# pgriewank/SAMSIM

Hardware: NVIDIA B200
Metric: column-timesteps/sec (FP64, 100 layers) (higher is better)
Workload: dtype f64

## Files before the change

samsim_b200/csrc/physics.cuh:

```cuda
#pragma once

#include <stdint.h>

#include "detmath.h"
#include "params.cuh"

namespace samsim {

struct DevCfg {
  int testcase;
  int Nlayer, N_top, N_middle, N_bottom;
  int atmoflux_flag, grav_flag, prescribe_flag, grav_heat_flag, flush_heat_flag, turb_flag, salt_flag,
      boundflux_flag, flush_flag, flood_flag, bottom_flag, precip_flag, harmonic_flag, tank_flag, albedo_flag,
      lab_snow_flag, freeboard_snow_flag, snow_flush_flag, snow_precip_flag;
  int i_time_out;
  int n_bgc;
  double dt, thick_0, thick_min, time_out;
  double alpha_flux_instable, alpha_flux_stable, m_total;
  double max_flux_plate, k_snow_flush, k_styropor;
  double c2, c3, c4, d2, d3x2, d4x3;
  int two_pass;
  int pf;
};

#ifdef SAMSIM_HOST_BUILD
static const DevCfg* samsim_host_cfg = nullptr;
#define CFG (*samsim::samsim_host_cfg)
#else
__constant__ DevCfg samsim_dev_cfg;
#define CFG samsim::samsim_dev_cfg
#endif

enum {
  SC_T_BOTTOM = 0, SC_T_TOP, SC_S_BU_BOTTOM, SC_T2M, SC_FL_Q_BOTTOM,
  SC_PSI_S_SNOW, SC_PSI_L_SNOW, SC_PSI_G_SNOW, SC_PHI_S, SC_S_ABS_SNOW, SC_H_ABS_SNOW, SC_M_SNOW, SC_T_SNOW,
  SC_THICK_SNOW, SC_LIQUID_PRECIP, SC_SOLID_PRECIP, SC_FL_Q_SNOW,
  SC_ENERGY_STORED, SC_TOTAL_RESIST, SC_FRESHWATER, SC_THICKNESS, SC_BULK_SALIN,
  SC_ALBEDO, SC_FL_SW, SC_FL_LW, SC_FL_REST,
  SC_GRAV_DRAIN, SC_GRAV_SALT, SC_GRAV_TEMP,
  SC_MELT_THICK, SC_MELT_THICK_SNOW, SC_MELT_THICK_SNOW_OLD,
  SC_MTO1, SC_MTO2, SC_MTO3,
  SC_FREEBOARD, SC_T_FREEZE, SC_MELT_ERR, SC_S_TOTAL,
  SC_TTOP_WARM, SC_TTOP_COLD, SC_OFLUX_AMP,
  SC_BGC_BOTTOM1, SC_BGC_BOTTOM2, SC_BGC_TOTAL1, SC_BGC_TOTAL2,
  SC_COUNT
};
enum {
  AR_M = 0, AR_S_ABS, AR_H_ABS, AR_THICK, AR_T, AR_PHI, AR_S_BU, AR_PSI_S, AR_PSI_L, AR_PSI_G, AR_RAY, AR_PERM,
  AR_FLUSH_V, AR_FLUSH_H, AR_FL_Q,
  AR_STATE_COUNT,
  AR_S_BR = AR_STATE_COUNT, AR_V_EX, AR_FL_M, AR_W0, AR_W1, AR_W2, AR_W3,
  AR_CORE_COUNT,
  AR_BGC1 = AR_CORE_COUNT, AR_BGC2, AR_FB_D, AR_FB_U, AR_FB_A, AR_FB_O,
  AR_COUNT
};
enum { IN_N_ACTIVE = 0, IN_STATUS, IN_STYROPOR, IN_EVENTS0, IN_EVENTS1, IN_COUNT };

enum {
  EV_FLOOD = 0, EV_FLOOD_NEG_FREE, EV_FLOOD_SIMPLE, EV_FLUSH3, EV_FLUSH4, EV_FLUSH_INLINE, EV_STYROPOR, EV_SNOW_THERMO,
  EV_SNOW_THERMO_MELTWATER, EV_SNOW_WET, EV_SNOW_MERGE, EV_SNOW_COMPACTION, EV_SNOW_COUPLING_ITER,
  EV_SNOW_COUPLING_WARM1, EV_SNOW_COUPLING_WARM2, EV_SNOW_PRECIP, EV_SNOW_PRECIP_0, EV_MELT_SNOW_ALL, EV_MELT_SNOW_PART,
  EV_BOTTOM_MELT, EV_BOTTOM_MELT_SIMPLE_A, EV_BOTTOM_MELT_SIMPLE_B, EV_BOTTOM_GROWTH_SIMPLE, EV_BOTTOM_GROWTH,
  EV_TOP_GROW_A, EV_TOP_GROW_B, EV_TOP_GROW_C, EV_TOP_MELT_A, EV_TOP_MELT_B, EV_TOP_MELT_C, EV_GRAV_DRAINED,
  EV_SALT_CLAMP,
  EV_GAS_REFILL, EV_GETT_TFR_FALLBACK, EV_GETT_SALTFREE, EV_GETT_LIQUID, EV_HEAT_MELT, EV_HEAT_THIN_SNOW,
  EV_MELT_THICK_GAS, EV_SNOW_MELTWATER_TO_ICE, EV_PRESCRIBE, EV_GRAV_DRAIN_SIMPLE, EV_NOTZFLUX, EV_FLUSH3_CLAMP,
  EV_SCRUB, EV_MELT_THICK, EV_TURB, EV_TANK, EV_TWO_PASS_STEP,
  EV_COUNT
};

struct Lay {
  double* p;
  unsigned ls;
  __device__ __forceinline__ double& operator[](int k) const {
#if !defined(SAMSIM_HOST_BUILD) && defined(__CUDA_ARCH__)
    __builtin_assume(__isGlobal(p));
#endif
    return p[(unsigned)k * ls];
  }
  __device__ __forceinline__ void prefetch(int k) const {
#ifndef SAMSIM_HOST_BUILD
    asm volatile("prefetch.global.L1 [%0];" ::"l"(p + (unsigned)k * ls));
#else
    (void)k;
#endif
  }
};
#ifndef SAMSIM_LOOP
#define SAMSIM_LOOP _Pragma("unroll 1")
#endif
#ifndef SAMSIM_PF
#define SAMSIM_PF (CFG.pf)
#endif

#define SAMSIM_TILE 32
struct View {
  double* base;
  unsigned ls;
  __device__ __forceinline__ Lay A(int id) const { return Lay{base + id * SAMSIM_TILE, ls}; }
  __device__ __forceinline__ Lay m() const { return A(AR_M); }
  __device__ __forceinline__ Lay S_abs() const { return A(AR_S_ABS); }
  __device__ __forceinline__ Lay H_abs() const { return A(AR_H_ABS); }
  __device__ __forceinline__ Lay thick() const { return A(AR_THICK); }
  __device__ __forceinline__ Lay T() const { return A(AR_T); }
  __device__ __forceinline__ Lay phi() const { return A(AR_PHI); }
  __device__ __forceinline__ Lay S_bu() const { return A(AR_S_BU); }
  __device__ __forceinline__ Lay psi_s() const { return A(AR_PSI_S); }
  __device__ __forceinline__ Lay psi_l() const { return A(AR_PSI_L); }
  __device__ __forceinline__ Lay psi_g() const { return A(AR_PSI_G); }
  __device__ __forceinline__ Lay ray() const { return A(AR_RAY); }
  __device__ __forceinline__ Lay perm() const { return A(AR_PERM); }
  __device__ __forceinline__ Lay flush_v() const { return A(AR_FLUSH_V); }
  __device__ __forceinline__ Lay flush_h() const { return A(AR_FLUSH_H); }
  __device__ __forceinline__ Lay fl_Q() const { return A(AR_FL_Q); }
  __device__ __forceinline__ Lay S_br() const { return A(AR_S_BR); }
  __device__ __forceinline__ Lay V_ex() const { return A(AR_V_EX); }
  __device__ __forceinline__ Lay fl_m() const { return A(AR_FL_M); }
  __device__ __forceinline__ Lay w0() const { return A(AR_W0); }
  __device__ __forceinline__ Lay w1() const { return A(AR_W1); }
  __device__ __forceinline__ Lay w2() const { return A(AR_W2); }
  __device__ __forceinline__ Lay w3() const { return A(AR_W3); }
  __device__ __forceinline__ Lay bgc(int q) const { return A(AR_BGC1 + q); }
};
struct Col : View {
  double fb_x;
  int N_active, status, styropor_flag;
  unsigned ev0, ev1;
  bool thermo_valid;
  bool want_state;
  struct FbMemo {
    bool tot_valid;  double t1, A, G;
    bool suf_valid;  int ks; double As, Gs;
    bool res_valid;  double m1, th1, msnow, result;
    int k_last;
  } fb;
  double min_psi_s, min_S_abs_2;
  struct Pre {
    bool valid;
    double mn2, sq2, st2;
    double bottom_h, S_br_Na, perm_Na;
    double A2;
  } pre;
  double sc[SC_COUNT];
  double time;
  long long i;
  int n_time_out, time_counter;
  double fsw0, fsw1, flw0, flw1;
  double ftime0, ftime1;
// ... 549 lines not shown
    m1 = m1 + m_snow;
    thick1 = thick1 + thick_snow;
    H_abs_snow = 0.0; m_snow = 0.0; thick_snow = 0.0;
    psi_g_snow = 0.0; psi_s_snow = 0.0; psi_l_snow = 0.0;
  }
  if (psi_g_snow < 0.0) c.status = 9876;
}

__device__ __forceinline__ void snow_block(Col& c) {
  const View v = c;
  if (SCV(c, SC_THICK_SNOW) > 0.0) {
    double m1 = v.m()[1], th1 = v.thick()[1], H1 = v.H_abs()[1];
    if (CFG.snow_flush_flag == 0) {
      double dummy = 0.0;
      snow_thermo(c, false, m1, th1, H1, dummy);
      SCV(c, SC_MELT_THICK_SNOW) = 0.0;
    } else if (CFG.snow_flush_flag == 1) {
      SCV(c, SC_MELT_THICK_SNOW) = 0.0;
      snow_thermo(c, true, m1, th1, H1, SCV(c, SC_MELT_THICK_SNOW));
    }
    v.m()[1] = m1; v.thick()[1] = th1; v.H_abs()[1] = H1;
  } else {
    SCV(c, SC_THICK_SNOW) = 0.0; SCV(c, SC_M_SNOW) = 0.0; SCV(c, SC_PSI_S_SNOW) = 0.0; SCV(c, SC_PSI_L_SNOW) = 0.0;
    SCV(c, SC_PSI_G_SNOW) = 0.0; SCV(c, SC_H_ABS_SNOW) = 0.0; SCV(c, SC_S_ABS_SNOW) = 0.0;
    SCV(c, SC_MELT_THICK_SNOW) = 0.0;
  }
}

__device__ __forceinline__ double fl_Q_0_snow_thin(double m_snow, double thick_snow, double T_snow, double ps,
                                                   double pl, double pg, double thick, double T_bound) {
  double ks = k_snow_of(m_snow, thick_snow);
  double k = ps * k_s + pl * k_l + pg * 0.0;
  k = thick_snow / (thick_snow + thick) * ks + thick / (thick_snow + thick) * k;
  double R = (thick_snow + thick) / (2.0 * k);
  return (T_snow - T_bound) / R;
}
__device__ __forceinline__ double fl_Q_snow_ice(double m_snow, double thick_snow, double T_snow, double ps2,
                                                double pl2, double th2, double T2) {
  double ks = k_snow_of(m_snow, thick_snow);
  double k2 = ps2 * k_s + pl2 * k_l;
  double R = thick_snow / (2.0 * ks) + th2 / (2.0 * k2);
  return (T2 - T_snow) / R;
}
__device__ __forceinline__ double fl_Q_0_snow(double m_snow, double thick_snow, double T_snow, double T_bound) {
  double k = k_snow_of(m_snow, thick_snow);
  double R = thick_snow / (2.0 * k);
  return (T_snow - T_bound) / R;
}


#ifndef SAMSIM_GB
#define SAMSIM_GB 8
#endif
__device__ __noinline__ void grav_drain(Col& c, bool exact_all) {
  const View v = c;
  const int Na = c.N_active, N = CFG.Nlayer;
  const double dt = CFG.dt;
  Lay q = v.w1(), smin = v.w2(), fl_m = v.fl_m();
  double heat_loss = 0.0;

  SAMSIM_LOOP
  for (int k = Na; k <= N - 1; k++) v.ray()[k] = 0.0;
  const double bottom_h = v.thick()[Na] * v.psi_s()[Na] / psi_s_min;
  const double S_br_Na = v.S_br()[Na];
  double perm_Na = 0.0;
  int kmin_cand = 0, ncand = 0;
  {
    double mn = 0.0, sq = 0.0, st = 0.0, st_below = 0.0, qb_est = 0.0;
    SAMSIM_LOOP
    for (int k = Na; k >= 1; k--) {
      if (k - SAMSIM_PF >= 1) { v.psi_l().prefetch(k - SAMSIM_PF); v.thick().prefetch(k - SAMSIM_PF); v.S_br().prefetch(k - SAMSIM_PF); }
      const double pk = 1e-17 * det_pow(1000.0 * fabs(v.psi_l()[k]), 3.10);
      if (k == Na) { perm_Na = pk; qb_est = bottom_h / pk; continue; }
      const double thk = v.thick()[k];
      const double qk = thk / pk;
      q[k] = qk;
      mn = (k == Na - 1) ? pk : f_min(mn, pk);
      if (exact_all) {
        smin[k] = mn;
      } else {
        st_below = st;
        sq = sq + qk;
        st = st + thk;
        double est;
        if (CFG.harmonic_flag == 1) {
          est = grav * rho_l * bbeta * (v.S_br()[k] - S_br_Na) * (st_below + bottom_h) * f_min(mn, perm_Na);
          smin[k] = mn;
        } else {
          const double hp = (mn < 1e-14) ? 0.0 : (st + bottom_h) / (sq + qb_est);
          est = grav * rho_l * bbeta * (v.S_br()[k] - S_br_Na) * (st_below + bottom_h) * hp;
        }
        est = est / (kappa_l * mu);
        const double rest = (CFG.harmonic_flag == 2 && mn < 1e-14) ? 0.0 : f_max(est, 0.0);
        v.ray()[k] = rest;
        if (rest > ray_crit * (1.0 - 1e-10)) { kmin_cand = k; ncand++; }
      }
    }
  }
  const double qb = bottom_h / perm_Na;

  const bool blocked = exact_all || ncand >= 3;
  const int kstop = exact_all ? 1 : kmin_cand;
  int kexact_from = exact_all ? 1 : Na;
  double carry_t = 0.0;
  for (int k0 = ((Na - 2) / SAMSIM_GB) * SAMSIM_GB + 1; blocked && k0 >= 1 && k0 + SAMSIM_GB - 1 >= kstop && Na >= 2; k0 -= SAMSIM_GB) {
    kexact_from = k0;
    double aq[SAMSIM_GB], at[SAMSIM_GB];
#pragma unroll
    for (int j = 0; j < SAMSIM_GB; j++) { aq[j] = 0.0; at[j] = 0.0; }
    SAMSIM_LOOP
    for (int d = 0; d < SAMSIM_GB; d++) {
      const int kk = k0 + d;
      if (kk <= Na - 1) {
        const double qv = q[kk], tv = v.thick()[kk];
#pragma unroll
        for (int j = 0; j < SAMSIM_GB; j++) {
          const double nq = aq[j] + qv, nt = at[j] + tv;
          aq[j] = (j <= d) ? nq : aq[j];
          at[j] = (j <= d) ? nt : at[j];
        }
      }
    }
    SAMSIM_LOOP
    for (int kk = k0 + SAMSIM_GB; kk <= Na - 1; kk++) {
      if (kk + 8 <= Na - 1) { q.prefetch(kk + 8); v.thick().prefetch(kk + 8); }
      const double qv = q[kk], tv = v.thick()[kk];
#pragma unroll
      for (int j = 0; j < SAMSIM_GB; j++) { aq[j] = aq[j] + qv; at[j] = at[j] + tv; }
    }
    const double carry_next = at[0];
    double below = carry_t;
    SAMSIM_LOOP
    for (int j = SAMSIM_GB - 1; j >= 0; j--) {
      const int k = k0 + j;
      const double aqj = aq[SAMSIM_GB - 1], atj = at[SAMSIM_GB - 1];
#pragma unroll
      for (int i = SAMSIM_GB - 1; i >= 1; i--) { aq[i] = aq[i - 1]; at[i] = at[i - 1]; }
      if (k <= Na - 1) {
        const double height = below + bottom_h;
        const double d_S_br = v.S_br()[k] - S_br_Na;
        double r;
        if (CFG.harmonic_flag == 1) {
          r = grav * rho_l * bbeta * d_S_br * height * f_min(smin[k], perm_Na);
        } else {
          const bool zero = exact_all ? (smin[k] < 1e-14) : (v.ray()[k] == 0.0);
          double hp;
          if (zero) {
            hp = 0.0;
          } else {
            hp = aqj + qb;
            hp = (atj + bottom_h) / hp;
          }
          r = grav * rho_l * bbeta * d_S_br * height * hp;
        }
        r = r / (kappa_l * mu);
        v.ray()[k] = f_max(r, 0.0);
      }
      below = atj;
    }
    carry_t = carry_next;
  }

  double sum_before = 0.0, sum_after = 0.0;
  double min_S = 1e300;
  int kfirst = 0;

  double run = 0.0;
  double sbk = v.S_br()[1];
  SAMSIM_LOOP
  for (int k = 1; k <= Na - 1; k++) {
    if (k + SAMSIM_PF <= Na) {
      v.ray().prefetch(k + SAMSIM_PF); v.S_abs().prefetch(k + SAMSIM_PF); v.S_br().prefetch(k + SAMSIM_PF);
    }
    double rk = v.ray()[k];
    const double Sk = v.S_abs()[k];
    const double sbk1 = v.S_br()[k + 1];
    if (k < kexact_from && rk > ray_crit * (1.0 - 1e-10)) {
      double hq = 0.0, ht = 0.0, hb = 0.0;
      SAMSIM_LOOP
      for (int kk = k; kk <= Na - 1; kk++) {
        const double tv = v.thick()[kk];
        hq = hq + q[kk];
        ht = ht + tv;
        if (kk > k) hb = hb + tv;
      }
      const double height = hb + bottom_h;
      const double d_S_br = sbk - S_br_Na;
      double r;
      if (CFG.harmonic_flag == 1) {
        r = grav * rho_l * bbeta * d_S_br * height * f_min(smin[k], perm_Na);
      } else {
        double hp = hq + qb;
        hp = (ht + bottom_h) / hp;
        r = grav * rho_l * bbeta * d_S_br * height * hp;
      }
      r = r / (kappa_l * mu);
      rk = f_max(r, 0.0);
      v.ray()[k] = rk;
    }
    double up = run;
    double S_after = Sk;
    double fl_down_k = 0.0;
    sum_before = sum_before + Sk;
    if (rk > ray_crit && v.psi_s()[k] > 0.001 && Sk / v.m()[k] > 0.1 && sbk > sbk1) {
      if (kfirst == 0) { kfirst = k; fl_m[k] = 0.0; EVT(c, EV_GRAV_DRAINED); }
      const double plk = v.psi_l()[k], thk = v.thick()[k], Tk = v.T()[k];
      double flux = x_grav * (rk - ray_crit) * dt * thk;
      flux = f_min(flux, plk * rho_l * thk);
      fl_down_k = flux;
      double Snew = Sk - flux * sbk;
      v.S_abs()[k] = Snew;
      S_after = Snew;
      if (Snew < 0.0) { c.status = 21234; return; }
      SCV(c, SC_GRAV_TEMP) = SCV(c, SC_GRAV_TEMP) + flux * Tk;
      v.H_abs()[k] = v.H_abs()[k] - flux * c_l * Tk;
      heat_loss = heat_loss + flux * c_l * Tk;
      run = run + flux;
      up = f_min(run, plk * rho_l * thk);
    }
    if (CFG.n_bgc) {
      const double cellNa = (k == Na - 1) ? v.A(AR_FB_D)[k] : v.A(AR_FB_A)[k];
      v.A(AR_FB_O)[k] = cellNa + fl_down_k;
      v.A(AR_FB_U)[k] = v.A(AR_FB_U)[k] + up;
    }
    if (kfirst) fl_m[k + 1] = up;
    else min_S = f_min(min_S, Sk);
    sum_after = sum_after + S_after;
    sbk = sbk1;
  }
  if (kfirst) fl_m[Na + 1] = run;
  if (CFG.n_bgc) v.A(AR_FB_U)[Na] = v.A(AR_FB_U)[Na] + run;
  const double fl_up_Na = run;
  {
    const double S_Na = v.S_abs()[Na];
    sum_before = sum_before + S_Na;
    sum_after = sum_after + S_Na;
  }
  SCV(c, SC_GRAV_SALT) = SCV(c, SC_GRAV_SALT) + sum_before;
  SCV(c, SC_GRAV_SALT) = SCV(c, SC_GRAV_SALT) - sum_after;

  if (kfirst) mass_transfer(c, fl_m, v.S_bu(), kfirst);

  SCV(c, SC_GRAV_DRAIN) = SCV(c, SC_GRAV_DRAIN) + run;
  if (CFG.grav_heat_flag == 2) v.H_abs()[Na] = v.H_abs()[Na] + heat_loss - fl_up_Na * c_l * SCV(c, SC_T_BOTTOM);
  double mn = min_S;
  if (kfirst) for (int k = kfirst; k <= Na; k++) mn = f_min(mn, v.S_abs()[k]);
  else mn = f_min(mn, v.S_abs()[Na]);
  if (f_min(mn, 0.0) < 0.0) c.status = 1337;
}

__device__ __noinline__ void grav_drain_simple(Col& c) {
  const View v = c;
  const int Na = c.N_active, N = CFG.Nlayer;
  Lay perm = v.w0(), hperm = v.w2();
  SAMSIM_LOOP
  for (int k = 1; k <= N - 1; k++) v.ray()[k] = 0.0;
  SAMSIM_LOOP
  for (int k = 1; k <= Na; k++) perm[k] = 1e-17 * det_pow(1000.0 * fabs(v.psi_l()[k]), 3.10);
  const double bottom_h = v.thick()[Na] * v.psi_s()[Na] / psi_s_min;
  if (CFG.harmonic_flag == 2) {
    SAMSIM_LOOP
    for (int k = 1; k <= Na - 1; k++) {
      double mn = perm[k];
      SAMSIM_LOOP
      for (int kk = k; kk <= Na - 1; kk++) mn = f_min(mn, perm[kk]);
      if (mn < 1e-14) {
        hperm[k] = 0.0;
      } else {
        double h = 0.0;
        SAMSIM_LOOP
        for (int kk = k; kk <= Na - 1; kk++) h = h + v.thick()[kk] / perm[kk];
        h = h + bottom_h / perm[Na];
        hperm[k] = (sum_fwd(v.thick(), k, Na - 1) + bottom_h) / h;
      }
    }
  }
  const double S_br_Na = v.S_br()[Na];
  SAMSIM_LOOP
  for (int k = 1; k <= Na - 1; k++) {
// ... 809 lines not shown
```

samsim_b200/csrc/samsim_b200.cu:

```cuda
#include <cuda_runtime.h>
#include <math.h>
#include <stdint.h>
#include <stdio.h>
#include <string.h>

#include <string>
#include <vector>

#include <cub/device/device_radix_sort.cuh>

#include "../../include/samsim_b200.h"
#include "step.cuh"

using namespace samsim;

static_assert((int)SAMSIM_SC_COUNT == (int)SC_COUNT, "scalar ids out of sync with include/samsim_b200.h");
static_assert((int)SAMSIM_ARR_COUNT == (int)AR_STATE_COUNT + 2 && (int)SAMSIM_ARR_BGC_ABS1 == (int)AR_STATE_COUNT,
              "array ids out of sync with include/samsim_b200.h");
static_assert((int)SAMSIM_INT_COUNT == (int)IN_COUNT, "int ids out of sync with include/samsim_b200.h");
static_assert((int)SAMSIM_EV_COUNT == (int)EV_COUNT && (int)SAMSIM_EV_TWO_PASS_STEP == (int)EV_TWO_PASS_STEP && (int)SAMSIM_EV_GAS_REFILL == 32,
              "event ids out of sync with include/samsim_b200.h");
static_assert((int)SAMSIM_SNAPSC_COUNT == 20 && (int)SAMSIM_SNAPARR_COUNT == 14, "snapshot layout");

#ifndef SAMSIM_BLOCK
// ... 34 lines not shown
  asm volatile("cp.async.ca.shared.global [%0], [%1], 8;\n" ::"r"(s), "l"(gmem_src));
}

template <bool TWO_PASS>
__global__ void __launch_bounds__(SAMSIM_BLOCK, SAMSIM_MINBLOCKS) samsim_step_kernel(const __grid_constant__ KParams p) {
  __shared__ double s_win[SAMSIM_MAXSITE * 4 * SAMSIM_MAXWIN];
  if (p.series != nullptr) {
    const int n = p.nsite * 4 * p.win_len;
    for (int e = threadIdx.x; e < n; e += blockDim.x) {
      const int sk = e / p.win_len, r = e - sk * p.win_len;
      cp_async8(&s_win[e], p.series + (size_t)sk * p.nrec + (p.win_first - 1 + r));
    }
    asm volatile("cp.async.commit_group;\n" ::);
    asm volatile("cp.async.wait_group 0;\n" ::);
  }
  __syncthreads();

  const long long col_raw = (long long)blockIdx.x * blockDim.x + threadIdx.x;
  const bool padding = (col_raw >= p.ncol);
  const long long col = padding ? (p.ncol - 1) : col_raw;
  const size_t ls = (size_t)p.ncol_pad;

  Col c;
  c.ls = (unsigned)(p.n_arr * SAMSIM_TILE);
  c.base = p.arr + (size_t)(col / SAMSIM_TILE) * p.LS * c.ls + (size_t)(col % SAMSIM_TILE);
  for (int q = 0; q < SC_COUNT; q++) c.sc[q] = p.sc[(size_t)q * ls + col];
  c.N_active = p.in[(size_t)IN_N_ACTIVE * ls + col];
  c.status = padding ? -1 : p.in[(size_t)IN_STATUS * ls + col];
  c.styropor_flag = p.in[(size_t)IN_STYROPOR * ls + col];
  c.ev0 = (unsigned)p.in[(size_t)IN_EVENTS0 * ls + col];
  c.ev1 = (unsigned)p.in[(size_t)IN_EVENTS1 * ls + col];
  c.time = p.time; c.i = p.i; c.n_time_out = p.n_time_out; c.time_counter = p.time_counter;
  c.fsw0 = c.fsw1 = c.flw0 = c.flw1 = c.ftime0 = c.ftime1 = 0.0;
  c.thermo_valid = false;
  c.pre.valid = false;
  c.want_state = false;
  c.fb.tot_valid = c.fb.suf_valid = c.fb.res_valid = false; c.fb.k_last = 0; c.fb.ks = 0;
  c.min_psi_s = 0.0; c.min_S_abs_2 = 0.0;
  c.fb_x = 0.0;

  Forcing f;
  f.win = s_win; f.win_len = p.win_len; f.win_first = p.win_first;
  f.site = p.site_of_col ? p.site_of_col[col] : 0;
  for (int k = 0; k < 4; k++) {
    f.scale[k] = p.fscale ? p.fscale[(size_t)k * ls + col] : 1.0;
    f.offset[k] = p.foffset ? p.foffset[(size_t)k * ls + col] : 0.0;
  }
  f.lab = p.lab; f.lab_nrec = p.lab_nrec;
  f.lab_set = p.set_of_col ? p.set_of_col[col] : 0;

  SnapOut snap;
  snap.scalars = p.snap_sc; snap.arrays = p.snap_arr; snap.ncol_pad = ls; snap.col = (int)col;

  for (int s = 0; s < p.nsteps; s++) column_step<TWO_PASS>(c, f, s == p.nsteps - 1, snap);

  if (p.divergence) {
    const unsigned full = 0xffffffffu;
    const bool live = !padding && c.status == 0;
    const int na = live ? c.N_active : 0;
    const int mx = __reduce_max_sync(full, na);
    const int idle = __reduce_add_sync(full, live ? (mx - na) : 0);
    const int nlive = __popc(__ballot_sync(full, live));
    const double ts = c.sc[SC_THICK_SNOW];
    const int cls = !live ? -1 : (((ts <= 0.0) ? 0 : (ts < CFG.thick_min / 100.0) ? 1 : (ts < CFG.thick_min) ? 2 : 3) |
                                  ((c.sc[SC_MELT_THICK] > 0.0) ? 4 : 0));
    const int cls0 = __shfl_sync(full, cls, __ffs(__ballot_sync(full, live)) - 1);
    const unsigned differ = __ballot_sync(full, live && cls != cls0);
    if ((threadIdx.x & 31) == 0 && nlive > 0) {
      atomicAdd(&p.divergence[0], (unsigned long long)idle);
      atomicAdd(&p.divergence[1], (unsigned long long)mx * (unsigned long long)nlive);
      atomicAdd(&p.divergence[2], (unsigned long long)(differ != 0u));
      atomicAdd(&p.divergence[3], 1ull);
    }
  }

  if (padding) return;
  for (int q = 0; q < SC_COUNT; q++) p.sc[(size_t)q * ls + col] = c.sc[q];
  p.in[(size_t)IN_N_ACTIVE * ls + col] = c.N_active;
  p.in[(size_t)IN_STATUS * ls + col] = c.status;
  p.in[(size_t)IN_STYROPOR * ls + col] = c.styropor_flag;
  p.in[(size_t)IN_EVENTS0 * ls + col] = (int)c.ev0;
  p.in[(size_t)IN_EVENTS1 * ls + col] = (int)c.ev1;
}

__device__ __forceinline__ long long slot_of(const int* map, long long col) { return map ? (long long)map[col] : col; }

__host__ __device__ __forceinline__ size_t state_index(long long s, int k, int a, int LS, int n_arr) {
  return ((((size_t)(s / SAMSIM_TILE)) * LS + k) * n_arr + a) * SAMSIM_TILE + (size_t)(s % SAMSIM_TILE);
}

__global__ void samsim_broadcast_kernel(double* arr, double* sc, int* in, long long ncol_pad, int LS, int src, int col0,
                                        int n, const int* map, int n_arr) {
  const long long t = (long long)blockIdx.x * blockDim.x + threadIdx.x;
  if (t >= n) return;
  const long long col = slot_of(map, col0 + t);
  src = (int)slot_of(map, src);
  if (col == src) return;
  const size_t ls = (size_t)ncol_pad;
  for (int k = 0; k < LS; k++)
    for (int a = 0; a < n_arr; a++) arr[state_index(col, k, a, LS, n_arr)] = arr[state_index(src, k, a, LS, n_arr)];
  for (int q = 0; q < SC_COUNT; q++) sc[(size_t)q * ls + col] = sc[(size_t)q * ls + src];
  for (int q = 0; q < IN_COUNT; q++) in[(size_t)q * ls + col] = in[(size_t)q * ls + src];
}

__global__ void samsim_gather_kernel(const double* src, double* dst, long long ncol_pad, int LS, int count, int ext,
                                     int col0, int n, int k0, const int* map) {
  const long long t = (long long)blockIdx.x * blockDim.x + threadIdx.x;
// ... 1064 lines not shown
  int rc = kat_common(device);
  if (rc) return rc;
  if (n < 1 || !a || !out) return fail(SAMSIM_ERR_ARG, "kat_scalar: bad argument");
  if ((rc = kat_upload_cfg(device, salt_flag))) return rc;
  double* d = nullptr;
  const size_t nb = (size_t)n * sizeof(double);
  CU(cudaMalloc(&d, 3 * nb));
  CU(cudaMemcpy(d, a, nb, cudaMemcpyHostToDevice));
  if (b) CU(cudaMemcpy(d + n, b, nb, cudaMemcpyHostToDevice));
  else CU(cudaMemset(d + n, 0, nb));
  samsim_kat_scalar_kernel<<<(n + 127) / 128, 128>>>(fn, salt_flag, n, d, d + n, d + 2 * (size_t)n);
  CU(cudaGetLastError());
  CU(cudaMemcpy(out, d + 2 * (size_t)n, nb, cudaMemcpyDeviceToHost));
  cudaFree(d);
  return 0;
}

int samsim_b200_fp64_peak(int32_t device, double seconds, double* tflops) {
  int rc = kat_common(device);
  if (rc) return rc;
  if (!tflops) return fail(SAMSIM_ERR_ARG, "fp64_peak: bad argument");
  cudaDeviceProp prop;
  CU(cudaGetDeviceProperties(&prop, device));
  const int blocks = prop.multiProcessorCount * 8, threads = 256;
  double* d = nullptr;
  CU(cudaMalloc(&d, (size_t)blocks * threads * sizeof(double)));
  cudaEvent_t e0, e1;
  cudaEventCreate(&e0);
  cudaEventCreate(&e1);
  int iters = 2000;
  double best = 0.0, elapsed_total = 0.0;
  samsim_fp64_peak_kernel<<<blocks, threads>>>(d, 100, 1.0);
  CU(cudaDeviceSynchronize());
  while (elapsed_total < seconds * 1000.0) {
    cudaEventRecord(e0);
    samsim_fp64_peak_kernel<<<blocks, threads>>>(d, iters, 1.0);
    cudaEventRecord(e1);
    CU(cudaEventSynchronize(e1));
    float ms = 0.f;
    cudaEventElapsedTime(&ms, e0, e1);
    elapsed_total += ms;
    const double flop = 2.0 * 64.0 * (double)iters * blocks * threads;
    const double tf = flop / (ms * 1e-3) / 1e12;
    if (tf > best) best = tf;
    if (ms < 50.f) iters *= 2;
  }
  cudaEventDestroy(e0);
  cudaEventDestroy(e1);
  cudaFree(d);
  *tflops = best;
  return 0;
}

}
```

samsim_b200/csrc/step.cuh:

```cuda
#pragma once

#include "physics.cuh"

namespace samsim {

struct Forcing {
  const double* win;
  int win_len;
  int win_first;
  int site;
  double scale[4], offset[4];
  const double* lab;
  long long lab_nrec;
  int lab_set;
};

__device__ __forceinline__ double forcing_rec(const Forcing& f, int kind, int rec ) {
  const double base = f.win[(f.site * 4 + kind) * f.win_len + (rec - f.win_first)];
  return base * f.scale[kind] + f.offset[kind];
}
__device__ __forceinline__ double time_input(int k) { return ((double)(float)k - 1.0) * 3600.0 * 3.0; }
__device__ __forceinline__ double lab_rec(const Forcing& f, int kind, long long rec ) {
  return f.lab[((long long)(f.lab_set * 4 + kind)) * f.lab_nrec + (rec - 1)];
}
// ... 201 lines not shown
      }
      double fq_kp1;
      double hr_n = 0.0, T_n = 0.0;
      if (k < Na) {
        const double ps_n = v.psi_s()[k + 1], pl_n = v.psi_l()[k + 1], th_n = v.thick()[k + 1];
        T_n = v.T()[k + 1];
        hr_n = th_n / (2.0 * (ps_n * k_s + pl_n * k_l + 0.0 * 0.0));
        const double R = hr_k + hr_n;
        fq_kp1 = (T_n - T_k) / R;
        if (c.want_state) v.fl_Q()[k + 1] = fq_kp1;
      } else {
        fq_kp1 = fl_q_bottom;
      }
      double H = v.H_abs()[k];
      temp1 = temp1 + H;
      H = H + (fq_kp1 - fq_k) * dt;
      H = H + rad;
      v.H_abs()[k] = H;
      temp2 = temp2 + H;
      fq_k = fq_kp1;
      hr_k = hr_n; T_k = T_n;
    }
    temp1 = temp1 + SCV(c, SC_H_ABS_SNOW);
    SAMSIM_LOOP
    for (int k = 1; k <= Na; k++) temp1 = temp1 + rad;
  }

  bool layer1_changed = false;
  if (thick_snow >= thick_min / 100.0 && thick_snow < thick_min) {
    EVT(c, EV_HEAT_THIN_SNOW);
    SCV(c, SC_H_ABS_SNOW) = SCV(c, SC_H_ABS_SNOW) - fl_q_snow * dt;
    double H1 = v.H_abs()[1], phi1 = v.phi()[1];
    snow_coupling(c, H1, phi1, T1, v.m()[1], v.S_bu()[1]);
    v.H_abs()[1] = H1; v.phi()[1] = phi1; v.T()[1] = T1;
    layer1_changed = true;
    temp1 = temp1 + fl_q_bottom * dt - fl_q_snow * dt;
  } else if (thick_snow >= thick_min) {
    SCV(c, SC_H_ABS_SNOW) = SCV(c, SC_H_ABS_SNOW) + (flQ1 - fl_q_snow) * dt;
    temp1 = temp1 + fl_q_bottom * dt - fl_q_snow * dt;
  } else {
    temp1 = temp1 + fl_q_bottom * dt - flQ1 * dt;
  }
  if (layer1_changed) temp2 = sum_fwd(v.H_abs(), 1, Na);
  temp2 = temp2 + SCV(c, SC_H_ABS_SNOW);
  if (fabs((temp1 - temp2) / dt) > 0.00001) c.status = 431;
}

#ifndef SAMSIM_SYNC
#define SAMSIM_SYNC 1
#endif
#ifndef SAMSIM_ALWAYS_STORE_S_BU
#define SAMSIM_ALWAYS_STORE_S_BU false
#endif
#if SAMSIM_SYNC
#define SAMSIM_PHASE_SYNC() __syncthreads()
#else
#define SAMSIM_PHASE_SYNC() ((void)0)
#endif
#if SAMSIM_SYNC >= 2
#error "SAMSIM_SYNC=2 (a barrier per layer of the Newton sweeps) was removed: it measured slower and its fused / unfused \
choice per thread made the barrier divergent (ADVICE round 1)"
#endif

struct SnapOut {
  double* scalars;
  double* arrays;
  size_t ncol_pad;
  int col;
};

__device__ __noinline__ void write_snapshot(const Col& c, const SnapOut& s) {
  const View v = c;
  if (s.scalars) {
    const int ids[19] = {SC_FREEBOARD, SC_THICK_SNOW, SC_T_SNOW, SC_PSI_L_SNOW, SC_PSI_S_SNOW, SC_ENERGY_STORED,
                         SC_FRESHWATER, SC_TOTAL_RESIST, SC_THICKNESS, SC_BULK_SALIN, SC_GRAV_DRAIN, SC_GRAV_SALT,
                         SC_GRAV_TEMP, SC_T2M, SC_T_TOP, SC_MTO1, SC_MTO2, SC_MTO3, -1};
    SAMSIM_LOOP
    for (int q = 0; q < 18; q++) s.scalars[(size_t)q * s.ncol_pad + s.col] = c.sc[ids[q]];
    s.scalars[(size_t)18 * s.ncol_pad + s.col] = c.time;
    s.scalars[(size_t)19 * s.ncol_pad + s.col] = (double)c.N_active;
  }
  if (s.arrays) {
    const int N = CFG.Nlayer;
    const size_t LS = (size_t)(N + 2);
    const int src[10] = {AR_T, AR_PSI_S, AR_THICK, AR_S_BU, AR_RAY, AR_PSI_L, AR_PERM, AR_FLUSH_V, AR_FLUSH_H, AR_PSI_G};
    SAMSIM_LOOP
    for (int a = 0; a < 10; a++) {
      double* dst = s.arrays + ((size_t)a * LS) * s.ncol_pad + s.col;
      const Lay from = v.A(src[a]);
      const int n = (a == 4) ? N - 1 : N;
      SAMSIM_LOOP
      for (int k = 1; k <= n; k++) dst[(size_t)k * s.ncol_pad] = from[k];
    }
    for (int q = 0; q < CFG.n_bgc; q++) {
      double* bu = s.arrays + ((size_t)(10 + 2 * q) * LS) * s.ncol_pad + s.col;
      double* br = s.arrays + ((size_t)(11 + 2 * q) * LS) * s.ncol_pad + s.col;
      const Lay x = v.bgc(q);
      const double bottom = c.sc[SC_BGC_BOTTOM1 + q];
      SAMSIM_LOOP
      for (int k = 1; k <= N; k++) {
        double vbu = bottom, vbr = bottom;
        if (k <= c.N_active) {
          const double mk = v.m()[k];
          if (mk != 0.0) {
            vbu = x[k] / mk;
            const double pl = v.psi_l()[k], th = v.thick()[k];
            vbr = (pl != 0.0 && th != 0.0) ? x[k] / pl / th / rho_l : 0.0;
          } else {
            vbu = 0.0; vbr = 0.0;
          }
        }
        bu[(size_t)k * s.ncol_pad] = vbu;
        br[(size_t)k * s.ncol_pad] = vbr;
      }
    }
  }
}

__device__ __noinline__ void fused_thermo_expulsion(Col& c) {
  const View v = c;
  const int Na = c.N_active;
  const bool transfer = (c.i != 1);
  {
    const double m1 = v.m()[1];
    const double sbu1 = v.S_abs()[1] / m1, H = v.H_abs()[1] / m1;
    double phi1 = v.phi()[1], T1;
    const double T_test = (Na >= 2) ? v.T()[2] : SCV(c, SC_T_BOTTOM);
    getT(H, sbu1, T_test, T1, phi1, c.status, c.ev1);
    v.T()[1] = T1; v.phi()[1] = phi1;
  }
  double T_km1 = 0.0, sbr_km1 = 0.0, Sabs_km1 = 0.0, f0 = 0.0;
  double fbA = 0.0, fbG = 0.0, fbAs = 0.0, fbGs = 0.0;
  const int ks = (c.fb.k_last >= 1 && c.fb.k_last < Na) ? c.fb.k_last : 0;
  double min_ps = 1e300;
  SAMSIM_LOOP
  for (int k = 1; k <= Na; k++) {
    if (k + SAMSIM_PF <= Na) {
      v.T().prefetch(k + SAMSIM_PF); v.phi().prefetch(k + SAMSIM_PF);
      v.m().prefetch(k + SAMSIM_PF); v.thick().prefetch(k + SAMSIM_PF); v.S_abs().prefetch(k + SAMSIM_PF);
      v.H_abs().prefetch(k + SAMSIM_PF);
    }
    const double thk = v.thick()[k], m_k = v.m()[k], T_k = v.T()[k];
    double S = v.S_abs()[k];
    const double sbr_k = S_br_of(T_k, S / m_k);
    v.S_br()[k] = sbr_k;
    double ps, pl, pg, vex;
    expulsion(v.phi()[k], thk, m_k, ps, pl, pg, vex);
    double f1;
    if (k == 1) {
      f1 = -vex * rho_l;
    } else if (pg < SAMSIM_F32(0.001)) {
      f1 = -vex * rho_l + f0;
    } else {
      f1 = -f_max((vex - pg * thk) * rho_l, 0.0);
      pg = f_max((pg * thk - vex) / thk, 0.0);
    }
    v.psi_s()[k] = ps; v.psi_l()[k] = pl; v.psi_g()[k] = pg;
    fbA = fbA + ps * thk;
    fbG = fbG + pg * thk;
    if (ks && k > ks) { fbAs = fbAs + ps * thk; fbGs = fbGs + pg * thk; }
    min_ps = f_min(min_ps, ps);
    const double m_new = m_k + f1 - f0;
    v.m()[k] = m_new;
    if (transfer) {
      double H = v.H_abs()[k];
      if (f1 < 0.) {
        H = H + f1 * T_k * c_l;
        S = S + f_max(f1 * sbr_k, -S);
      }
      if (f0 < 0) {
        H = H - f0 * T_km1 * c_l;
        S = S - f_max(f0 * sbr_km1, -Sabs_km1);
      }
      v.H_abs()[k] = H;
      v.S_abs()[k] = S;
    }
    v.S_bu()[k] = S / m_new;
    if (CFG.n_bgc) {
      v.A(AR_FB_D)[k] = transfer ? -f1 : 0.0;
      v.A(AR_FB_U)[k] = 0.0; v.A(AR_FB_A)[k] = 0.0; v.A(AR_FB_O)[k] = 0.0;
    }
    T_km1 = T_k; sbr_km1 = sbr_k; Sabs_km1 = S;
    f0 = f1;
  }
  c.fb.tot_valid = true; c.fb.t1 = v.thick()[1]; c.fb.A = fbA; c.fb.G = fbG;
  c.fb.suf_valid = (ks != 0); c.fb.ks = ks; c.fb.As = fbAs; c.fb.Gs = fbGs;
  c.fb.res_valid = false;
  c.min_psi_s = min_ps;
}

__device__ __forceinline__ void testcase_hooks(Col& c, const Forcing& f) {
  const View v = c;
  const double dt = CFG.dt;
  const int N = CFG.Nlayer;
  if (CFG.testcase == 1) {
    const double j = rint(c.time / 43200.0);
    if (j >= 1.0 && j <= 20.0 && fabs(c.time - 12.0 * j * 3600.0) < SAMSIM_F32(0.01))
      SCV(c, SC_T_TOP) = (((int)j) & 1) ? SCV(c, SC_TTOP_COLD) : SCV(c, SC_TTOP_WARM);
  } else if (CFG.testcase >= 101 && CFG.testcase <= 105) {
    const long long idx = (long long)floor(1 + c.time / dt);
    const double Sb = v.S_bu()[c.N_active + 1];
    SCV(c, SC_T2M) = lab_rec(f, 0, idx);
    SCV(c, SC_SOLID_PRECIP) = lab_rec(f, 1, idx);
    SCV(c, SC_FL_Q_BOTTOM) = lab_rec(f, 2, idx);
    SCV(c, SC_T_BOTTOM) = -SAMSIM_F32(0.0575) * Sb + SAMSIM_F32(1.710523e-3) * det_pow(Sb, 3.0 / 2.0) -
                          SAMSIM_F32(2.154996e-4) * P2(Sb) - SAMSIM_F32(7.53e-4) * sum_fwd(v.thick(), 1, c.N_active - 1);
    c.styropor_flag = (int)lab_rec(f, 3, idx);
  } else if (CFG.testcase == 4 || CFG.testcase == 7) {
    const double amp = SCV(c, SC_OFLUX_AMP);
    SCV(c, SC_FL_Q_BOTTOM) = -amp * det_sin(c.time * (2.0 * pi_sp) / (86400.0 * 365.0)) + amp;
  } else if (CFG.testcase == 2) {
    if (c.time > 86400.0 * 25.0) SCV(c, SC_T2M) = 15.0;
    else if (c.time > 86400.0 * 15.0) SCV(c, SC_T2M) = 1.0;
  } else if (CFG.testcase == 9) {
    if (c.time < (19.75 * 3600.0)) SCV(c, SC_T2M) = 0.0;
    else if (c.time < (86400.0 * 3.0 + 2.25 * 3600.0)) SCV(c, SC_T2M) = -15.0;
    else SCV(c, SC_T2M) = 1.0;
  } else if (CFG.testcase == 34) {
    if (c.time < 2.0 * 3600.0) SCV(c, SC_T2M) = 0.0;
    else if (c.time < (86400.0 * 5.0)) SCV(c, SC_T2M) = -15.0;
    else if (c.time < (86400.0 * 7.0)) SCV(c, SC_T2M) = -5.0;
    else SCV(c, SC_T2M) = 1.0;
  } else if (CFG.testcase == 99) {
    if (c.time < 86400.0 * 3.0) {
      SCV(c, SC_T2M) = -40.0;
    } else {
      SCV(c, SC_T2M) = (c.time > 86400.0 * 5.0) ? 5.0 : -5.0;
      SCV(c, SC_THICK_SNOW) = 0.2;
      SCV(c, SC_T_SNOW) = -5.0;
      SCV(c, SC_M_SNOW) = 30.0;
// ... 405 lines not shown
        double fq_jp1, hr_n = 0.0, T_n = 0.0;
        if (j < Na) {
          const double ps_n = v.psi_s()[j + 1], pl_n = v.psi_l()[j + 1], th_n = v.thick()[j + 1];
          T_n = v.T()[j + 1];
          hr_n = th_n / (2.0 * (ps_n * k_s + pl_n * k_l + 0.0 * 0.0));
          fq_jp1 = (T_n - T_j) / (hr_j + hr_n);
        } else {
          fq_jp1 = fl_q_bottom;
        }
        double Hh = v.H_abs()[j];
        temp1 = temp1 + Hh;
        Hh = Hh + (fq_jp1 - fq_km1) * dt;
        Hh = Hh + rad;
        v.H_abs()[j] = Hh;
        temp2 = temp2 + Hh;
        fq_km1 = fq_jp1; hr_j = hr_n; T_j = T_n;
      }
    }
  }

  c.fb.tot_valid = true; c.fb.t1 = v.thick()[1]; c.fb.A = fbA; c.fb.G = fbG;
  c.fb.suf_valid = (ks != 0); c.fb.ks = ks; c.fb.As = fbAs; c.fb.Gs = fbGs;
  c.fb.res_valid = false;
  c.min_psi_s = neg_ps ? -1.0 : 1.0;

  if (!merge_heat) {
    if (c.status == 0) heat_fluxes(c);
    return;
  }
  v.fl_Q()[1] = flQ1;
  v.fl_Q()[Na + 1] = fl_q_bottom;
  temp1 = temp1 + SCV(c, SC_H_ABS_SNOW);
  SAMSIM_LOOP
  for (int kk = 1; kk <= Na; kk++) temp1 = temp1 + rad;
  if (SCV(c, SC_THICK_SNOW) >= CFG.thick_min) {
    const double fl_q_snow = SCV(c, SC_FL_Q_SNOW);
    SCV(c, SC_H_ABS_SNOW) = SCV(c, SC_H_ABS_SNOW) + (flQ1 - fl_q_snow) * dt;
    temp1 = temp1 + fl_q_bottom * dt - fl_q_snow * dt;
  } else {
    temp1 = temp1 + fl_q_bottom * dt - flQ1 * dt;
  }
  temp2 = temp2 + SCV(c, SC_H_ABS_SNOW);
  if (c.status == 0 && fabs((temp1 - temp2) / dt) > 0.00001) c.status = 431;
}

template <bool TWO_PASS>
__device__ __noinline__ void column_step(Col& c, const Forcing& f, bool want_diag, const SnapOut& snap) {
  const View v = c;
  const double dt = CFG.dt;
  const int N = CFG.Nlayer;
  c.i = c.i + 1;
  c.want_state = want_diag;
  const bool output_step = (c.n_time_out == CFG.i_time_out || c.i == 1);

  if (c.status == 0) {
  if (output_step || want_diag) vital_signs(c);

  if (CFG.atmoflux_flag == 2) {
    if (c.time > time_input(c.time_counter)) c.time_counter = c.time_counter + 1;
    const int tc = c.time_counter;
    c.ftime1 = time_input(tc);
    c.fsw1 = forcing_rec(f, 0, tc);
    c.flw1 = forcing_rec(f, 1, tc);
    if (c.time == c.ftime1) {
      SCV(c, SC_T2M) = forcing_rec(f, 2, tc);
      SCV(c, SC_LIQUID_PRECIP) = forcing_rec(f, 3, tc);
      c.ftime0 = 0.0; c.fsw0 = 0.0; c.flw0 = 0.0;
    } else {
      c.ftime0 = time_input(tc - 1);
      c.fsw0 = forcing_rec(f, 0, tc - 1);
      c.flw0 = forcing_rec(f, 1, tc - 1);
      const double temp = (c.time - c.ftime0) / (c.ftime1 - c.ftime0);
      SCV(c, SC_T2M) = (1.0 - temp) * forcing_rec(f, 2, tc - 1) + temp * forcing_rec(f, 2, tc);
      SCV(c, SC_LIQUID_PRECIP) = (1.0 - temp) * forcing_rec(f, 3, tc - 1) + temp * forcing_rec(f, 3, tc);
    }
  }
  long long lab_idx = 0;
  if (CFG.boundflux_flag == 3 && CFG.lab_snow_flag == 1) {
    lab_idx = (long long)floor(1 + c.time / dt);
    SCV(c, SC_SOLID_PRECIP) = lab_rec(f, 1, lab_idx);
  }

  {
    const double lp = SCV(c, SC_LIQUID_PRECIP), sp = SCV(c, SC_SOLID_PRECIP);
    if (f_max(lp, sp) > 0.0 && (CFG.precip_flag == 1 || CFG.precip_flag == 0)) {
      const bool have_solid = (CFG.precip_flag == 0);
      if (c.N_active > 1) {
        EVT(c, EV_SNOW_PRECIP);
        snow_precip(c, dt, lp, SCV(c, SC_T2M), have_solid, sp);
      } else if (c.N_active == 1) {
        EVT(c, EV_SNOW_PRECIP_0);
        double H1 = v.H_abs()[1], S1 = v.S_abs()[1];
        snow_precip_0(H1, S1, v.m()[1], v.T()[1], dt, lp, SCV(c, SC_T2M), have_solid, sp);
        v.H_abs()[1] = H1; v.S_abs()[1] = S1;
      }
    }
  }

  snow_block(c);

  }
  SAMSIM_PHASE_SYNC();
  const bool next_step_outputs_pre = ((output_step ? 0 : c.n_time_out + 1) == CFG.i_time_out);
  const bool fast = TWO_PASS && (c.status == 0) && fast_path_ok(c, output_step, want_diag || next_step_outputs_pre);
  if (c.status == 0 && !fast) {
  if (!c.thermo_valid) backward_pass<false>(c, false, false);
  fused_thermo_expulsion(c);

  }
  SAMSIM_PHASE_SYNC();
  if (c.status == 0) {
  c.fb_x = 0.0;
  if (output_step) {
    SCV(c, SC_FREEBOARD) = (c.N_active > 1) ? freeboard_of(c) : 0.0;
    if (CFG.grav_flag == 2) {
      if (SCV(c, SC_GRAV_DRAIN) == 0.0) SCV(c, SC_GRAV_TEMP) = 0.0;
      else SCV(c, SC_GRAV_TEMP) = SCV(c, SC_GRAV_TEMP) / SCV(c, SC_GRAV_DRAIN);
      SCV(c, SC_GRAV_SALT) = SCV(c, SC_GRAV_SALT) / CFG.time_out;
      SCV(c, SC_GRAV_DRAIN) = SCV(c, SC_GRAV_DRAIN) / CFG.time_out;
    }
    write_snapshot(c, snap);
    SCV(c, SC_GRAV_DRAIN) = 0.0; SCV(c, SC_GRAV_SALT) = 0.0; SCV(c, SC_GRAV_TEMP) = 0.0;
    SCV(c, SC_MTO1) = 0.0; SCV(c, SC_MTO2) = 0.0; SCV(c, SC_MTO3) = 0.0;
    c.n_time_out = 0;
  } else {
    c.n_time_out = c.n_time_out + 1;
  }

  }
  SAMSIM_PHASE_SYNC();
  if (c.status == 0 && !fast) {
  {
    const int Na = c.N_active;
    const double pg = v.psi_g()[Na];
    if (pg > 0.0) {
      EVT(c, EV_GAS_REFILL);
      const double temp2 = pg * v.thick()[Na] * rho_l;
      c.fb.res_valid = false;
      v.m()[Na] = v.m()[Na] + temp2;
      v.S_abs()[Na] = v.S_abs()[Na] + temp2 * SCV(c, SC_S_BU_BOTTOM);
      v.H_abs()[Na] = v.H_abs()[Na] + temp2 * c_l * SCV(c, SC_T_BOTTOM);
    }
  }

  if (SCV(c, SC_M_SNOW) > 0.0 && SCV(c, SC_THICK_SNOW) < CFG.thick_min) {
    double H1 = v.H_abs()[1], phi1 = v.phi()[1], T1 = v.T()[1];
    snow_coupling(c, H1, phi1, T1, v.m()[1], v.S_bu()[1]);
    v.H_abs()[1] = H1; v.phi()[1] = phi1; v.T()[1] = T1;
    }

  if (c.N_active > 1 && CFG.flood_flag > 1) {
    SCV(c, SC_FREEBOARD) = freeboard_of(c);
    if (SCV(c, SC_FREEBOARD) < 0.0) {
      if (CFG.flood_flag == 2) { flood(c); fb_reset(c); }
      else if (CFG.flood_flag == 3 && SCV(c, SC_FREEBOARD) < neg_free) { flood_simple(c); fb_reset(c); }
    }
  }

  if (CFG.turb_flag == 2) {
    EVT(c, EV_TURB);
    const int Na = c.N_active;
    const double S = v.S_abs()[Na], mNa = v.m()[Na];
    const double turb = Turb_A * det_exp(Turb_B * (-density_of(SCV(c, SC_T_BOTTOM), SCV(c, SC_S_BU_BOTTOM)) + density_of(v.T()[Na], S / mNa))) * dt;
    v.S_abs()[Na] = S - turb * (S / mNa - SCV(c, SC_S_BU_BOTTOM));
    for (int q = 0; q < CFG.n_bgc; q++) {
      const double b = v.bgc(q)[Na];
      v.bgc(q)[Na] = b - turb * (b / mNa - SCV(c, SC_BGC_BOTTOM1 + q));
    }
  }

  }
  SAMSIM_PHASE_SYNC();
  if (TWO_PASS) {
    if (c.status == 0 && fast) {
      EVT(c, EV_TWO_PASS_STEP);
      testcase_hooks(c, f);
      forward_pass(c);
    }
  }
  if (c.status == 0 && !fast) {
  if (CFG.grav_flag == 2 && c.N_active > 1) {
    const bool next_step_outputs = (c.n_time_out == CFG.i_time_out);
    grav_drain(c, c.want_state || next_step_outputs);
  }
  else if (CFG.grav_flag == 3 && c.N_active > 1) { EVT(c, EV_GRAV_DRAIN_SIMPLE); grav_drain_simple(c); }

  if (CFG.prescribe_flag == 2) {
    EVT(c, EV_PRESCRIBE);
    const int Na = c.N_active;
    const double Sb = SCV(c, SC_S_BU_BOTTOM);
    int k = Na;
    while (k > 1 && sum_fwd(v.thick(), k, Na) < 0.15) {
      v.S_bu()[k] = Sb - sum_fwd(v.thick(), k, Na) / 0.15 * (Sb - 4.0);
      k = k - 1;
    }
    while (k > 1 && sum_fwd(v.thick(), k, Na) >= 0.15) {
      v.S_bu()[k] = 4.0 - 4.0 * (sum_fwd(v.thick(), k, Na) - 0.15) / (sum_fwd(v.thick(), 1, Na) - 0.15);
      k = k - 1;
      v.S_bu()[1] = 0.0;
    }
    v.S_bu()[Na] = Sb;
    SAMSIM_LOOP
    for (int kk = 1; kk <= N; kk++) v.S_abs()[kk] = v.S_bu()[kk] * v.m()[kk];
  }

  }
  SAMSIM_PHASE_SYNC();
  if (c.status == 0 && !fast) {
  testcase_hooks(c, f);

  if (CFG.tank_flag == 2) {
    EVT(c, EV_TANK);
    SCV(c, SC_S_BU_BOTTOM) = (SCV(c, SC_S_TOTAL) - sum_fwd(v.S_abs(), 1, c.N_active)) / (CFG.m_total - sum_fwd(v.m(), 1, c.N_active));
    if (CFG.n_bgc) {
      const double vb = (SCV(c, SC_BGC_TOTAL1) - sum_fwd(v.bgc(0), 1, c.N_active)) / (CFG.m_total - sum_fwd(v.m(), 1, c.N_active));
      for (int q = 0; q < CFG.n_bgc; q++) SCV(c, SC_BGC_BOTTOM1 + q) = vb;
    }
  }

  heat_fluxes(c);

  }
  SAMSIM_PHASE_SYNC();
  if (c.status == 0) {
  {
    const bool next_step_outputs = (c.n_time_out == CFG.i_time_out);
    const bool prepare = TWO_PASS && !(c.want_state || next_step_outputs) && c.N_active >= 3 && CFG.grav_flag == 2 &&
                         CFG.harmonic_flag == 2 && CFG.n_bgc == 0;
    backward_pass<TWO_PASS>(c, prepare, c.want_state || SAMSIM_ALWAYS_STORE_S_BU);
  }

  }
  SAMSIM_PHASE_SYNC();
  if (c.status == 0) {
  SCV(c, SC_MELT_THICK_SNOW_OLD) = SCV(c, SC_MELT_THICK_SNOW);
  snow_block(c);
// ... 130 lines not shown
```

Before: 120.5 million.

## Defer S_bu stores to grav_drain and skip undrained layers in flux loop

Outside output, prescribe and bgc steps, fused_thermo_expulsion no longer writes bulk salinity for interior layers. grav_drain writes S_bu only for layers from the first drained one downward, which cuts per-layer global stores. When there are no bgc tracers, grav_drain also runs a light loop over layers above the lowest Rayleigh candidate that only accumulates salt sums, skipping ray/S_br loads. The change also adds optional phase-cycle and host traffic-count instrumentation behind compile flags. The risk is that S_bu is left stale in undrained interior layers, which is correct only if nothing reads it before the next output step.

```diff
diff --git a/samsim_b200/csrc/physics.cuh b/samsim_b200/csrc/physics.cuh
--- a/samsim_b200/csrc/physics.cuh
+++ b/samsim_b200/csrc/physics.cuh
@@ -69,15 +69,33 @@
   EV_COUNT
 };
 
+#if defined(SAMSIM_HOST_BUILD) && defined(SAMSIM_COUNT_TRAFFIC)
+#define SAMSIM_TRAFFIC_PHASES 16
+static const double* samsim_traffic_base = nullptr;
+static int samsim_traffic_phase = 0;
+static long long samsim_traffic[SAMSIM_TRAFFIC_PHASES][AR_COUNT][2];
+inline void samsim_traffic_count(const double* e, int w);
+struct LayRef {
+  double* e;
+  operator double() const { samsim_traffic_count(e, 0); return *e; }
+  const LayRef& operator=(double x) const { samsim_traffic_count(e, 1); *e = x; return *this; }
+  const LayRef& operator=(const LayRef& o) const { return *this = (double)o; }
+};
+#endif
+
 struct Lay {
   double* p;
   unsigned ls;
+#if defined(SAMSIM_HOST_BUILD) && defined(SAMSIM_COUNT_TRAFFIC)
+  LayRef operator[](int k) const { return LayRef{p + (unsigned)k * ls}; }
+#else
   __device__ __forceinline__ double& operator[](int k) const {
 #if !defined(SAMSIM_HOST_BUILD) && defined(__CUDA_ARCH__)
     __builtin_assume(__isGlobal(p));
 #endif
     return p[(unsigned)k * ls];
   }
+#endif
   __device__ __forceinline__ void prefetch(int k) const {
 #ifndef SAMSIM_HOST_BUILD
     asm volatile("prefetch.global.L1 [%0];" ::"l"(p + (unsigned)k * ls));
@@ -94,6 +112,13 @@
 #endif
 
 #define SAMSIM_TILE 32
+#if defined(SAMSIM_HOST_BUILD) && defined(SAMSIM_COUNT_TRAFFIC)
+inline void samsim_traffic_count(const double* e, int w) {
+  const long long off = (e - samsim_traffic_base) / SAMSIM_TILE;
+  const int ph = samsim_traffic_phase < SAMSIM_TRAFFIC_PHASES ? samsim_traffic_phase : SAMSIM_TRAFFIC_PHASES - 1;
+  if (samsim_traffic_base && off >= 0) samsim_traffic[ph][off % AR_COUNT][w]++;
+}
+#endif
 struct View {
   double* base;
   unsigned ls;
@@ -749,7 +774,7 @@
 #ifndef SAMSIM_GB
 #define SAMSIM_GB 8
 #endif
-__device__ __noinline__ void grav_drain(Col& c, bool exact_all) {
+__device__ __noinline__ void grav_drain(Col& c, bool exact_all, bool store_S_bu) {
   const View v = c;
   const int Na = c.N_active, N = CFG.Nlayer;
   const double dt = CFG.dt;
@@ -797,10 +822,10 @@
   const double qb = bottom_h / perm_Na;
 
   const bool blocked = exact_all || ncand >= 3;
-  const int kstop = exact_all ? 1 : kmin_cand;
+  const int kc = exact_all ? 1 : (ncand ? kmin_cand : Na);
   int kexact_from = exact_all ? 1 : Na;
   double carry_t = 0.0;
-  for (int k0 = ((Na - 2) / SAMSIM_GB) * SAMSIM_GB + 1; blocked && k0 >= 1 && k0 + SAMSIM_GB - 1 >= kstop && Na >= 2; k0 -= SAMSIM_GB) {
+  for (int k0 = ((Na - 2) / SAMSIM_GB) * SAMSIM_GB + 1; blocked && k0 >= 1 && k0 + SAMSIM_GB - 1 >= kc && Na >= 2; k0 -= SAMSIM_GB) {
     kexact_from = k0;
     double aq[SAMSIM_GB], at[SAMSIM_GB];
 #pragma unroll
@@ -863,9 +888,20 @@
   int kfirst = 0;
 
   double run = 0.0;
-  double sbk = v.S_br()[1];
-  SAMSIM_LOOP
-  for (int k = 1; k <= Na - 1; k++) {
+  int k = 1;
+  if (CFG.n_bgc == 0) {
+    SAMSIM_LOOP
+    for (; k < kc; k++) {
+      if (k + SAMSIM_PF <= Na) v.S_abs().prefetch(k + SAMSIM_PF);
+      const double Sk = v.S_abs()[k];
+      sum_before = sum_before + Sk;
+      min_S = f_min(min_S, Sk);
+      sum_after = sum_after + Sk;
+    }
+  }
+  double sbk = v.S_br()[k];
+  SAMSIM_LOOP
+  for (; k <= Na - 1; k++) {
     if (k + SAMSIM_PF <= Na) {
       v.ray().prefetch(k + SAMSIM_PF); v.S_abs().prefetch(k + SAMSIM_PF); v.S_br().prefetch(k + SAMSIM_PF);
     }
@@ -900,7 +936,10 @@
     double fl_down_k = 0.0;
     sum_before = sum_before + Sk;
     if (rk > ray_crit && v.psi_s()[k] > 0.001 && Sk / v.m()[k] > 0.1 && sbk > sbk1) {
-      if (kfirst == 0) { kfirst = k; fl_m[k] = 0.0; EVT(c, EV_GRAV_DRAINED); }
+      if (kfirst == 0) {
+        kfirst = k; fl_m[k] = 0.0; EVT(c, EV_GRAV_DRAINED);
+        if (store_S_bu && k - 1 >= 2) v.S_bu()[k - 1] = v.S_abs()[k - 1] / v.m()[k - 1];
+      }
       const double plk = v.psi_l()[k], thk = v.thick()[k], Tk = v.T()[k];
       double flux = x_grav * (rk - ray_crit) * dt * thk;
       flux = f_min(flux, plk * rho_l * thk);
@@ -920,8 +959,12 @@
       v.A(AR_FB_O)[k] = cellNa + fl_down_k;
       v.A(AR_FB_U)[k] = v.A(AR_FB_U)[k] + up;
     }
-    if (kfirst) fl_m[k + 1] = up;
-    else min_S = f_min(min_S, Sk);
+    if (kfirst) {
+      fl_m[k + 1] = up;
+      if (store_S_bu && k >= 2) v.S_bu()[k] = Sk / v.m()[k];
+    } else {
+      min_S = f_min(min_S, Sk);
+    }
     sum_after = sum_after + S_after;
     sbk = sbk1;
   }
diff --git a/samsim_b200/csrc/samsim_b200.cu b/samsim_b200/csrc/samsim_b200.cu
--- a/samsim_b200/csrc/samsim_b200.cu
+++ b/samsim_b200/csrc/samsim_b200.cu
@@ -110,7 +110,19 @@
   SnapOut snap;
   snap.scalars = p.snap_sc; snap.arrays = p.snap_arr; snap.ncol_pad = ls; snap.col = (int)col;
 
+#if defined(SAMSIM_PHASE_CLOCK) && SAMSIM_SYNC
+  if (threadIdx.x == 0) {
+    for (int q = 0; q < SAMSIM_NPHASE; q++) samsim_pc_acc[q] = 0;
+    samsim_pc_ph = 0;
+  }
+  __syncthreads();
+  if (threadIdx.x == 0) samsim_pc_t0 = clock64();
+#endif
   for (int s = 0; s < p.nsteps; s++) column_step<TWO_PASS>(c, f, s == p.nsteps - 1, snap);
+#if defined(SAMSIM_PHASE_CLOCK) && SAMSIM_SYNC
+  if (threadIdx.x == 0)
+    for (int q = 0; q < SAMSIM_NPHASE; q++) atomicAdd(&samsim_phase_cycles[q], samsim_pc_acc[q]);
+#endif
 
   if (p.divergence) {
     const unsigned full = 0xffffffffu;
@@ -1281,4 +1293,15 @@
   return 0;
 }
 
-}
+#if defined(SAMSIM_PHASE_CLOCK) && SAMSIM_SYNC
+int samsim_b200_phase_cycles(unsigned long long* out) {
+  if (!out) return fail(SAMSIM_ERR_ARG, "phase_cycles: bad argument");
+  CU(cudaDeviceSynchronize());
+  CU(cudaMemcpyFromSymbol(out, samsim_phase_cycles, sizeof(unsigned long long) * SAMSIM_NPHASE));
+  const unsigned long long zero[SAMSIM_NPHASE] = {};
+  CU(cudaMemcpyToSymbol(samsim_phase_cycles, zero, sizeof zero));
+  return SAMSIM_NPHASE;
+}
+#endif
+
+}
diff --git a/samsim_b200/csrc/step.cuh b/samsim_b200/csrc/step.cuh
--- a/samsim_b200/csrc/step.cuh
+++ b/samsim_b200/csrc/step.cuh
@@ -277,7 +277,25 @@
 #ifndef SAMSIM_ALWAYS_STORE_S_BU
 #define SAMSIM_ALWAYS_STORE_S_BU false
 #endif
-#if SAMSIM_SYNC
+#define SAMSIM_NPHASE 9
+#if defined(SAMSIM_HOST_BUILD) && defined(SAMSIM_COUNT_TRAFFIC)
+#define SAMSIM_PHASE_SYNC() (samsim_traffic_phase = (samsim_traffic_phase + 1) % SAMSIM_NPHASE)
+#elif defined(SAMSIM_PHASE_CLOCK) && SAMSIM_SYNC
+__device__ unsigned long long samsim_phase_cycles[SAMSIM_NPHASE];
+__shared__ unsigned long long samsim_pc_acc[SAMSIM_NPHASE];
+__shared__ long long samsim_pc_t0;
+__shared__ int samsim_pc_ph;
+#define SAMSIM_PHASE_SYNC()                                                                 \
+  do {                                                                                      \
+    __syncthreads();                                                                        \
+    if (threadIdx.x == 0) {                                                                 \
+      const long long t_ = clock64();                                                       \
+      samsim_pc_acc[samsim_pc_ph] += (unsigned long long)(t_ - samsim_pc_t0);               \
+      samsim_pc_t0 = t_;                                                                    \
+      samsim_pc_ph = (samsim_pc_ph + 1 == SAMSIM_NPHASE) ? 0 : samsim_pc_ph + 1;            \
+    }                                                                                       \
+  } while (0)
+#elif SAMSIM_SYNC
 #define SAMSIM_PHASE_SYNC() __syncthreads()
 #else
 #define SAMSIM_PHASE_SYNC() ((void)0)
@@ -342,10 +360,11 @@
   }
 }
 
-__device__ __noinline__ void fused_thermo_expulsion(Col& c) {
+__device__ __noinline__ void fused_thermo_expulsion(Col& c, bool s7_all) {
   const View v = c;
   const int Na = c.N_active;
   const bool transfer = (c.i != 1);
+  const unsigned nskip = s7_all ? 0u : (unsigned)(Na - 2);
   {
     const double m1 = v.m()[1];
     const double sbu1 = v.S_abs()[1] / m1, H = v.H_abs()[1] / m1;
@@ -400,7 +419,7 @@
       v.H_abs()[k] = H;
       v.S_abs()[k] = S;
     }
-    v.S_bu()[k] = S / m_new;
+    if ((unsigned)(k - 2) >= nskip) v.S_bu()[k] = S / m_new;
     if (CFG.n_bgc) {
       v.A(AR_FB_D)[k] = transfer ? -f1 : 0.0;
       v.A(AR_FB_U)[k] = 0.0; v.A(AR_FB_A)[k] = 0.0; v.A(AR_FB_O)[k] = 0.0;
@@ -912,6 +931,7 @@
   c.i = c.i + 1;
   c.want_state = want_diag;
   const bool output_step = (c.n_time_out == CFG.i_time_out || c.i == 1);
+  const bool s7_all = output_step || CFG.prescribe_flag == 2 || CFG.n_bgc != 0;
 
   if (c.status == 0) {
   if (output_step || want_diag) vital_signs(c);
@@ -965,7 +985,7 @@
   const bool fast = TWO_PASS && (c.status == 0) && fast_path_ok(c, output_step, want_diag || next_step_outputs_pre);
   if (c.status == 0 && !fast) {
   if (!c.thermo_valid) backward_pass<false>(c, false, false);
-  fused_thermo_expulsion(c);
+  fused_thermo_expulsion(c, s7_all);
 
   }
   SAMSIM_PHASE_SYNC();
@@ -1041,7 +1061,7 @@
   if (c.status == 0 && !fast) {
   if (CFG.grav_flag == 2 && c.N_active > 1) {
     const bool next_step_outputs = (c.n_time_out == CFG.i_time_out);
-    grav_drain(c, c.want_state || next_step_outputs);
+    grav_drain(c, c.want_state || next_step_outputs, !s7_all);
   }
   else if (CFG.grav_flag == 3 && c.N_active > 1) { EVT(c, EV_GRAV_DRAIN_SIMPLE); grav_drain_simple(c); }
 
```

New measurement: 124.3 million, median of 6. +3.2%, better.
